# falfab/orb_slam_cuda

Measured on AMD Instinct MI355X. Metric: frames/s ORB extract+match, 1241×376 mono nFeatures=2000; achieved HBM GB/s, higher is better.
Workload: dtype u8

## Files before the change

### orb_slam_cuda_amd/csrc/orbx_blur.hip

```cpp
#include "orbx_device.cuh"

namespace orbx {

#ifndef ORBX_BLUR_TH
#define ORBX_BLUR_TH 48
#endif
#ifndef ORBX_BLUR_TW
#define ORBX_BLUR_TW 128
#endif
constexpr int kBlurTWs = 64, kBlurTHs = 32;

typedef unsigned short us2_t __attribute__((ext_vector_type(2)));
__device__ __forceinline__ uint32_t dot4(uint32_t px, uint32_t taps, uint32_t acc) {
  return __builtin_amdgcn_udot4(px, taps, acc, false);
}
__device__ __forceinline__ uint32_t dot2(uint32_t pair, uint32_t taps, uint32_t acc) {
  return __builtin_amdgcn_udot2(__builtin_bit_cast(us2_t, pair), __builtin_bit_cast(us2_t, taps), acc, false);
}

template <int kBlurTW, int kBlurTH>
__global__ __launch_bounds__(256) void blur_kernel(ExtractParams P, LevelPtrs lp, const int2* __restrict__ rtab,
                                                   int tiles, int ntiles, unsigned magic, uint8_t* __restrict__ blur) {
  constexpr int kBlurInW = kBlurTW + 32;
  constexpr int kBlurPairs = (kBlurTH + 6 + 1) / 2;
  __shared__ __attribute__((aligned(16))) uint8_t in[kBlurPairs * 2][kBlurInW];
  __shared__ __attribute__((aligned(16))) uint32_t tmp[kBlurPairs][kBlurTW];
  const int wg = xcd_remap(blockIdx.x + blockIdx.y * gridDim.x, gridDim.x * gridDim.y);
  const int f = magic ? (int)__umulhi((unsigned)wg, magic) : wg / ntiles, tid = threadIdx.x;
  const int e = rtab[tiles + wg - f * ntiles].x;
  const int l = e & 15, x0 = (e >> 4) & 0xFFF, y0 = e >> 16;
  const LevelGeom& g = P.lv[l];
  const int W = g.w, H = g.h;
  const uint8_t* S = lp.base[l] + f * lp.fstride[l];
  const int pitch = lp.pitch[l];
  typedef unsigned int u32x4 __attribute__((ext_vector_type(4)));
  constexpr int kChunks = kBlurInW / 16, kItems = (kBlurTH + 6) * kChunks, kPer = (kItems + 255) / 256;
  if (lp.aligned16[l]) {
    const int xmax = min(pitch, (W + 15) & ~15) - 16;
    u32x4 v[kPer];
#pragma unroll
    for (int q = 0; q < kPer; ++q) {
      const int i = min(tid + 256 * q, kItems - 1);
      const int r = i / kChunks, ch = i - r * kChunks;
      const int gy = reflect101(min(max(y0 + r - 3, -(H - 1)), 2 * H - 2), H);
      const int gx = min(max(x0 - 16 + ch * 16, 0), xmax);
      v[q] = *(const u32x4*)(S + (long long)gy * pitch + gx);
    }
#pragma unroll
    for (int q = 0; q < kPer; ++q) {
      const int i = min(tid + 256 * q, kItems - 1);
      const int r = i / kChunks, ch = i - r * kChunks;
      *(u32x4*)&in[r][ch * 16] = v[q];
    }
    const bool left = x0 == 0, right = x0 + kBlurTW + 3 > W;
    if (left || right) {
      __syncthreads();
      for (int i = tid; i < (kBlurTH + 6) * 6; i += 256) {
        const int r = i / 6, kk = i - r * 6;
        int x = kk < 3 ? -1 - kk : W + kk - 3;
        if ((kk < 3 && !left) || (kk >= 3 && !right) || x - x0 + 16 >= kBlurInW) continue;
        in[r][x - x0 + 16] = in[r][reflect101(x, W) - x0 + 16];
      }
    }
  } else {
    u32x4 v[kPer];
    bool direct[kPer];
    int gys[kPer];
#pragma unroll
    for (int q = 0; q < kPer; ++q) {
      const int i = min(tid + 256 * q, kItems - 1);
      const int r = i / kChunks, ch = i - r * kChunks;
      gys[q] = reflect101(min(max(y0 + r - 3, -(H - 1)), 2 * H - 2), H);
      const int gx = x0 - 16 + ch * 16;
      const uint8_t* src = S + (long long)gys[q] * pitch + gx;
      direct[q] = gx >= 0 && gx + 16 <= W && (((uintptr_t)src) & 15) == 0;
      v[q] = *(const u32x4*)(direct[q] ? src : S);
    }
#pragma unroll
    for (int q = 0; q < kPer; ++q) {
      const int i = min(tid + 256 * q, kItems - 1);
      const int r = i / kChunks, ch = i - r * kChunks;
      *(u32x4*)&in[r][ch * 16] = v[q];
    }
#pragma unroll
    for (int q = 0; q < kPer; ++q) {
      if (direct[q]) continue;
      const int i = min(tid + 256 * q, kItems - 1);
      const int r = i / kChunks, ch = i - r * kChunks;
      const int gx = x0 - 16 + ch * 16;
      const uint8_t* src = S + (long long)gys[q] * pitch;
#pragma unroll
      for (int k = 0; k < 16; ++k) {
        const int xx = min(max(gx + k, -(W - 1)), 2 * W - 2);
        in[r][ch * 16 + k] = src[reflect101(xx, W)];
      }
    }
  }
  __syncthreads();
  const int* k = P.gauss;
  const uint32_t kA0 = (k[0] << 8) | (k[1] << 16) | (k[2] << 24), kB0 = k[3] | (k[4] << 8) | (k[5] << 16) | (k[6] << 24);
  const uint32_t kA1 = (k[0] << 16) | (k[1] << 24), kB1 = k[2] | (k[3] << 8) | (k[4] << 16) | (k[5] << 24), kC1 = k[6];
  const uint32_t kA2 = k[0] << 24, kB2 = k[1] | (k[2] << 8) | (k[3] << 16) | (k[4] << 24), kC2 = k[5] | (k[6] << 8);
  const uint32_t kB3 = k[0] | (k[1] << 8) | (k[2] << 16) | (k[3] << 24), kC3 = k[4] | (k[5] << 8) | (k[6] << 16);
  const int opairs = (min(kBlurTH, H - y0) + 1) >> 1;
  for (int i = tid; i < min(kBlurPairs, opairs + 3) * (kBlurTW / 4); i += 256) {
    const int pr = i / (kBlurTW / 4), x = (i - pr * (kBlurTW / 4)) * 4;
    uint32_t o[2][4];
#pragma unroll
    for (int h = 0; h < 2; ++h) {
      const uint32_t* row = (const uint32_t*)in[2 * pr + h];
      const uint32_t A = row[(x + 12) >> 2], B = row[(x + 16) >> 2], C = row[(x + 20) >> 2];
      o[h][0] = dot4(B, kB0, dot4(A, kA0, 0));
      o[h][1] = dot4(C, kC1, dot4(B, kB1, dot4(A, kA1, 0)));
      o[h][2] = dot4(C, kC2, dot4(B, kB2, dot4(A, kA2, 0)));
      o[h][3] = dot4(C, kC3, dot4(B, kB3, 0));
    }
    *(uint4*)&tmp[pr][x] = make_uint4(o[0][0] | (o[1][0] << 16), o[0][1] | (o[1][1] << 16),
                                      o[0][2] | (o[1][2] << 16), o[0][3] | (o[1][3] << 16));
  }
  __syncthreads();
  const uint32_t t01 = k[0] | (k[1] << 16), t23 = k[2] | (k[3] << 16), t45 = k[4] | (k[5] << 16), t6 = k[6];
  const uint32_t u0 = k[0] << 16, u12 = k[1] | (k[2] << 16), u34 = k[3] | (k[4] << 16), u56 = k[5] | (k[6] << 16);
  uint8_t* D = blur + g.off + f * g.plane;
  for (int i = tid; i < opairs * (kBlurTW / 4); i += 256) {
    const int rp = i / (kBlurTW / 4), cx = (i - rp * (kBlurTW / 4)) * 4;
    const uint4 q0 = *(const uint4*)&tmp[rp][cx], q1 = *(const uint4*)&tmp[rp + 1][cx];
    const uint4 q2 = *(const uint4*)&tmp[rp + 2][cx], q3 = *(const uint4*)&tmp[rp + 3][cx];
    const uint32_t P0[4] = {q0.x, q0.y, q0.z, q0.w}, P1[4] = {q1.x, q1.y, q1.z, q1.w};
    const uint32_t P2[4] = {q2.x, q2.y, q2.z, q2.w}, P3[4] = {q3.x, q3.y, q3.z, q3.w};
    int va[4], vb[4];
#pragma unroll
    for (int q = 0; q < 4; ++q) {
      const uint32_t a = dot2(P3[q], t6, dot2(P2[q], t45, dot2(P1[q], t23, dot2(P0[q], t01, 1u << 15))));
      const uint32_t b = dot2(P3[q], u56, dot2(P2[q], u34, dot2(P1[q], u12, dot2(P0[q], u0, 1u << 15))));
      va[q] = min((int)(a >> 16), 255);
      vb[q] = min((int)(b >> 16), 255);
    }
    const uint32_t pa = pack4_u8(va[0], va[1], va[2], va[3]), pb = pack4_u8(vb[0], vb[1], vb[2], vb[3]);
    const int x = x0 + cx;
#pragma unroll
    for (int h = 0; h < 2; ++h) {
      const int y = y0 + 2 * rp + h;
      if (y >= H) break;
      const uint32_t packed = h ? pb : pa;
      uint8_t* dst = D + (long long)y * g.pitch + x;
      if (x + 4 <= W) {
        *(uint32_t*)dst = packed;
      } else {
        for (int q = 0; q < 4 && x + q < W; ++q) dst[q] = (uint8_t)(packed >> (8 * q));
      }
    }
  }
}

void blur_tile_dims(int small, int* tw, int* th) {
  *tw = small ? kBlurTWs : ORBX_BLUR_TW;
  *th = small ? kBlurTHs : ORBX_BLUR_TH;
}

int launch_blur(const ExtractParams& P, const LevelPtrs& lp, const int2* rtab, uint8_t* blur, int batch,
                hipStream_t s) {
  static const int cus = [] {
    int dev = 0, n = 256;
    (void)hipGetDevice(&dev);
    (void)hipDeviceGetAttribute(&n, hipDeviceAttributeMultiprocessorCount, dev);
    return n;
  }();
  if ((long long)P.blur_ntiles[0] * batch >= 2ll * cus)
    hipLaunchKernelGGL((blur_kernel<ORBX_BLUR_TW, ORBX_BLUR_TH>), dim3(P.blur_ntiles[0], batch), dim3(256), 0, s, P,
                       lp, rtab, P.blur_tiles[0], P.blur_ntiles[0], P.blur_magic[0], blur);
  else
    hipLaunchKernelGGL((blur_kernel<kBlurTWs, kBlurTHs>), dim3(P.blur_ntiles[1], batch), dim3(256), 0, s, P, lp,
                       rtab, P.blur_tiles[1], P.blur_ntiles[1], P.blur_magic[1], blur);
  return hipGetLastError() == hipSuccess ? ORBX_OK : ORBX_EDEVICE;
}

}
```

### orb_slam_cuda_amd/csrc/orbx_host.hip

```cpp
#include <hip/hip_runtime.h>

#include <algorithm>
#include <atomic>
#include <chrono>
#include <condition_variable>
#include <cfloat>
#include <cstdarg>
#include <climits>
#include <cmath>
#include <cstdio>
#include <cstdlib>
#include <cstring>
#include <mutex>
#include <string>
#include <thread>
#include <vector>

#include "orbx_internal.h"
#include "orbx_sincosf.h"

namespace orbx {

__global__ __launch_bounds__(256) void copy2d_kernel(uint8_t* __restrict__ d, size_t dp, const uint8_t* __restrict__ s,
                                                     size_t sp, size_t w, size_t rows) {
  const size_t cpr = (w + 15) / 16, total = cpr * rows;
  for (size_t i = blockIdx.x * 256ull + threadIdx.x; i < total; i += (size_t)gridDim.x * 256) {
    const size_t r = i / cpr, c = (i - r * cpr) * 16;
    const uint8_t* src = s + r * sp + c;
    uint8_t* dst = d + r * dp + c;
    if (c + 16 <= w) {
      *(uint4*)dst = *(const uint4*)src;
    } else {
      for (size_t k = 0; k < 16 && c + k < w; ++k) dst[k] = src[k];
    }
  }
}
size_t quadtree_lds_bytes(const ExtractParams& P);
size_t quadtree_legacy_lds_bytes(const ExtractParams& P);
size_t quadtree_sorted_lds_bytes(const ExtractParams& P, int big);
int quadtree_sorted_ownmax(const ExtractParams& P, int big, size_t budget);
extern const void* quadtree_kernel_ptr(const ExtractParams& P);
size_t pyr_band_lds_bytes(const ExtractParams& P);
void blur_tile_dims(int small, int* tw, int* th);
extern const void* pyr_band_kernel_ptr();
extern int pyr_band_occupancy(size_t lds);
}

using namespace orbx;

static size_t out_desc_off(int cap_frame) { return (16 + (size_t)cap_frame * sizeof(orbx_kp) + 15) & ~(size_t)15; }

static thread_local std::string g_err;
static int fail(int code, const char* fmt, ...) {
  char buf[512];
  va_list ap;
  va_start(ap, fmt);
  vsnprintf(buf, sizeof buf, fmt, ap);
  va_end(ap);
  g_err = buf;
  return code;
}
#define HIP_OK(expr)                                                                        \
  do {                                                                                      \
    hipError_t e_ = (expr);                                                                 \
    if (e_ != hipSuccess) return fail(ORBX_EDEVICE, "%s: %s", #expr, hipGetErrorString(e_)); \
  } while (0)

namespace {

inline int cv_round(float v) { return (int)lrintf(v); }
inline int cv_floor(float v) { int i = (int)v; return i - (i > v); }
inline short sat_short(int v) { return (short)std::min(std::max(v, (int)SHRT_MIN), (int)SHRT_MAX); }

struct DeviceBuf {
  void* p = nullptr;
  size_t n = 0;
  ~DeviceBuf() { if (p) (void)hipFree(p); }
  int alloc(size_t bytes) {
    if (p) { (void)hipFree(p); p = nullptr; }
    n = bytes;
    if (!bytes) return ORBX_OK;
    if (hipMalloc(&p, bytes) != hipSuccess) return fail(ORBX_ENOMEM, "hipMalloc(%zu) failed", bytes);
    return ORBX_OK;
  }
  template <class T> T* as() const { return (T*)p; }
};

struct Plan {
  int W = 0, H = 0, B = 0;
  ExtractParams P{};
  std::vector<CellGeom> cells;
  std::vector<int2> rtab;
  DeviceBuf pyr, blur, rtab_d, cells_d, umax_d, slots, cell_counts, qkeys, qcounts, qties, qscratch, qnscratch,
      err;
};

}

struct orbx_extractor {
  orbx_config cfg{};
  std::vector<float> scale, inv_scale, sigma2, inv_sigma2;
  std::vector<int> nfeat;
  int umax[16];
  Plan plan;
  hipStream_t stream = nullptr;
  DeviceBuf d_in, d_out;
  void* h_in = nullptr;
  void* h_out = nullptr;
  size_t h_in_bytes = 0, h_out_bytes = 0;
  hipGraphExec_t graph = nullptr;
  int graph_w = 0, graph_h = 0;
  bool graph_hp = false;
  bool last_single = false;
  bool last_empty = false;
  int warm_w = 0, warm_h = 0;
  int last_batch = 0;
  const uint8_t* last_frames = nullptr;
  size_t last_fpitch = 0, last_rstride = 0;
  bool timing = false;
  hipEvent_t ev[6] = {};
  void* user_ev[ORBX_STAGE_EVENTS] = {};
  bool has_user_ev = false;
  WsOrder ws;
  bool host_pyr = false;
  bool host_pyr_valid = false;
  void* h_pyr = nullptr;
  size_t h_pyr_bytes = 0;
  long long h_pyr_off[kMaxLevels] = {};
  hipStream_t pstream = nullptr;
  hipEvent_t pev[2] = {};
  std::vector<float> prof_t[4];
  char order[6] = {};
  std::mutex mu;
};

WsOrder* orbx::extractor_ws(orbx_handle h) { return h ? &h->ws : nullptr; }

static void compute_scales(orbx_extractor* h) {
  const orbx_config& c = h->cfg;
  const int L = c.nlevels;
  h->scale.assign(L, 1.f);
  h->sigma2.assign(L, 1.f);
  for (int i = 1; i < L; i++) {
    h->scale[i] = h->scale[i - 1] * c.scale_factor;
    h->sigma2[i] = h->scale[i] * h->scale[i];
  }
  h->inv_scale.resize(L);
  h->inv_sigma2.resize(L);
  for (int i = 0; i < L; i++) {
    h->inv_scale[i] = 1.0f / h->scale[i];
    h->inv_sigma2[i] = 1.0f / h->sigma2[i];
  }
  h->nfeat.assign(L, 0);
  const float factor = 1.0f / c.scale_factor;
  float nDesired = c.nfeatures * (1 - factor) / (1 - (float)pow((double)factor, (double)L));
  int sum = 0;
  for (int l = 0; l < L - 1; l++) {
    h->nfeat[l] = cv_round(nDesired);
    sum += h->nfeat[l];
    nDesired *= factor;
  }
  h->nfeat[L - 1] = std::max(c.nfeatures - sum, 0);
  const int HP = kHalfPatch;
  int v, v0;
  const int vmax = cv_floor(HP * sqrtf(2.f) / 2 + 1);
  const int vmin = (int)std::ceil(HP * sqrtf(2.f) / 2);
  const double hp2 = HP * HP;
  for (v = 0; v <= vmax; ++v) h->umax[v] = (int)lrint(sqrt(hp2 - v * v));
  for (v = HP, v0 = 0; v >= vmin; --v) {
    while (h->umax[v0] == h->umax[v0 + 1]) ++v0;
    h->umax[v] = v0;
    ++v0;
  }
  if (c.scale_mode == ORBX_SCALE_F) {
    for (int l = 0; l < L; ++l) {
      const unsigned vw = (unsigned)std::ceil(c.width * std::pow(0.8408964, l));
      h->scale[l] = ((float)c.width) / vw;
      h->inv_scale[l] = ((float)vw) / c.width;
    }
  }
}

static void gaussian7(int k[7]) {
  float cf[7];
  double sum = 0;
  for (int i = 0; i < 7; ++i) {
    const double x = i - 3.0;
    cf[i] = (float)std::exp(-0.5 / (2.0 * 2.0) * x * x);
    sum += cf[i];
  }
  sum = 1. / sum;
  for (int i = 0; i < 7; ++i) cf[i] = (float)(cf[i] * sum);
  for (int i = 0; i < 7; ++i) k[i] = cv_round(cf[i] * 256.f);
}

static void resize_tables(int sw, int sh, int dw, int dh, std::vector<int2>& xt, std::vector<int2>& yt,
// ... 241 lines not shown
      code |= (uint32_t)bit << (2 * (Dh - 1 - j) + 1);
    }
    t[(size_t)g.boxW + y] = code;
  }
  *bits = (Dh << 8) | ((R + 2 * Dh) << 16);
  return true;
}

static int build_plan(orbx_extractor* h, int W, int Hh, int B) {
  Plan& pl = h->plan;
  const orbx_config& c = h->cfg;
  const int L = c.nlevels;
  ExtractParams P{};
  P.L = L;
  P.B = B;
  const int ini = std::min(std::max(c.ini_th_fast, 0), 255), mn = std::min(std::max(c.min_th_fast, 0), 255);
  P.t_ini = ini;
  P.t_min = mn;
  P.t_low = std::min(ini, mn);
  P.pattern_upstream = c.pattern_mode == ORBX_PATTERN_UPSTREAM;
  gaussian7(P.gauss);
  pl.cells.clear();
  pl.rtab.clear();
  long long lvl_off = 0;
  int slot = 0, kbase = 0, maxnodes = 0, maxcells = 0;
  for (int l = 0; l < L; ++l) {
    LevelGeom& g = P.lv[l];
    const float inv = h->inv_scale[l];
    g.w = cv_round((float)W * inv);
    g.h = cv_round((float)Hh * inv);
    if (g.w > kMaxLevelDim || g.h > kMaxLevelDim)
      return fail(ORBX_EINVAL, "level %d is %dx%d; at most %d px per side", l, g.w, g.h, kMaxLevelDim);
    g.pitch = (g.w + 63) & ~63;
    g.plane = (long long)g.h * g.pitch;
    g.minBX = kEdgeThreshold - 3;
    g.minBY = g.minBX;
    g.maxBX = g.w - kEdgeThreshold + 3;
    g.maxBY = g.h - kEdgeThreshold + 3;
    const float width = (float)(g.maxBX - g.minBX), height = (float)(g.maxBY - g.minBY);
    g.nCols = (int)(width / kGridW);
    g.nRows = (int)(height / kGridW);
    if (g.nCols < 1 || g.nRows < 1)
      return fail(ORBX_EINVAL,
                  "level %d (%dx%d) is smaller than one %d-px FAST cell inside the %d-px border; "
                  "the reference divides by zero here (src/ORBextractor.cc:1144-1147)",
                  l, g.w, g.h, kGridW, kEdgeThreshold);
    g.wCell = (int)std::ceil(width / g.nCols);
    g.hCell = (int)std::ceil(height / g.nRows);
    if (g.wCell + 6 > kMaxRoi - 1 || g.hCell + 6 > kMaxRoi - 1)
      return fail(ORBX_EINVAL, "level %d cell %dx%d exceeds the ROI tile", l, g.wCell, g.hCell);
    g.cell0 = (int)pl.cells.size();
    g.slot0 = slot;
    for (int i = 0; i < g.nRows; i++) {
      const float iniY = g.minBY + i * g.hCell;
      float maxY = iniY + g.hCell + 6;
      const bool skipRow = iniY >= g.maxBY - 3;
      if (maxY > g.maxBY) maxY = g.maxBY;
      for (int j = 0; j < g.nCols; j++) {
        const float iniX = g.minBX + j * g.wCell;
        float maxX = iniX + g.wCell + 6;
        const bool skip = skipRow || iniX >= g.maxBX - 6;
        if (maxX > g.maxBX) maxX = g.maxBX;
        CellGeom cg{};
        cg.level = (int16_t)l;
        cg.c0 = (int16_t)(int)iniX;
        cg.r0 = (int16_t)(int)iniY;
        cg.c1 = (int16_t)(int)maxX;
        cg.r1 = (int16_t)(int)maxY;
        const int bw = cg.c1 - cg.c0 - 6, bh = cg.r1 - cg.r0 - 6;
        cg.cap = (skip || bw <= 0 || bh <= 0) ? 0 : (int16_t)(((bw + 1) / 2) * ((bh + 1) / 2));
        if (cg.cap) {
          P.fast_rh_max = std::max(P.fast_rh_max, cg.r1 - cg.r0);
          P.fast_bw_max = std::max(P.fast_bw_max, bw);
          P.fast_bh_max = std::max(P.fast_bh_max, bh);
        }
        cg.pitch = l == 0 ? 0 : g.pitch;
        cg.row_off = l == 0 ? cg.r0 : (int)(lvl_off + (long long)cg.r0 * g.pitch);
        cg.fstride = l == 0 ? 0 : (int)g.plane;
        cg.geo = (g.h - 1 - cg.r0) | (((g.w + 15) & ~15) << 16);
        pl.cells.push_back(cg);
      }
    }
    g.ncells = (int)pl.cells.size() - g.cell0;
    int stride = 1;
    for (int c = g.cell0; c < (int)pl.cells.size(); ++c) stride = std::max(stride, (int)pl.cells[c].cap);
    for (int c = g.cell0; c < (int)pl.cells.size(); ++c) pl.cells[c].slot_off = slot + (c - g.cell0) * stride;
    g.slot_stride = stride;
    slot += g.ncells * stride;
    g.nslots = slot - g.slot0;
    maxcells = std::max(maxcells, g.ncells);
    g.N = h->nfeat[l];
    g.boxW = g.maxBX - g.minBX;
    g.boxH = g.maxBY - g.minBY;
    g.nIni = (int)roundf(static_cast<float>(g.boxW) / g.boxH);
    if (g.nIni < 1) return fail(ORBX_EINVAL, "level %d: nIni = 0 (image taller than 1.5x its width)", l);
    g.hX = static_cast<float>(g.boxW) / g.nIni;
    g.kcap = std::max(g.N + 3, g.nIni);
    g.kbase = kbase;
    kbase += (g.kcap + kKpGroup - 1) / kKpGroup * kKpGroup;
    maxnodes = std::max(maxnodes, g.kcap + 4);
    g.scale = h->scale[l];
    g.size = (float)(int)(kPatchSize * h->scale[l]);
    g.off = lvl_off;
    lvl_off += (long long)B * g.plane;
    if (l >= 1) {
      std::vector<int2> xt, yt;
      resize_tables(P.lv[l - 1].w, P.lv[l - 1].h, g.w, g.h, xt, yt, &g.xmax, &g.area2x);
      for (int x0 = 0; x0 < g.w; x0 += 256) {
        const int xe = std::min(x0 + 255, g.w - 1);
        const int lo = g.area2x ? 2 * x0 : xt[x0].x, hi = g.area2x ? 2 * xe + 1 : xt[xe].x + 1;
        if (hi - (lo & ~15) + 16 > 576)
          return fail(ORBX_EINVAL, "scaleFactor %g too large for the pyramid tile (max 2.0)", c.scale_factor);
      }
      for (int y0 = 0; y0 < g.h; y0 += 16) {
        const int ye = std::min(y0 + 15, g.h - 1);
        const int lo = g.area2x ? 2 * y0 : (yt[y0].x & 0xFFFF), hi = g.area2x ? 2 * ye + 1 : (yt[ye].x >> 16);
        if (hi - lo + 1 > 36)
          return fail(ORBX_EINVAL, "scaleFactor %g too large for the pyramid tile (max 2.0)", c.scale_factor);
      }
      g.xtab = (int)pl.rtab.size();
      pl.rtab.insert(pl.rtab.end(), xt.begin(), xt.end());
      g.ytab = (int)pl.rtab.size();
      pl.rtab.insert(pl.rtab.end(), yt.begin(), yt.end());
      g.xtab2 = (int)pl.rtab.size();
      for (int dx = 0; dx < g.w; ++dx) {
        int2 e = xt[dx];
        if (g.area2x) e = make_int2(2 * dx, 0);
        else if (dx >= g.xmax) e.y = 2048;
        pl.rtab.push_back(e);
      }
    }
  }
  P.qt_tabmax = 0;
  P.qt_nbmax = 0;
  for (int l = 0; l < L; ++l) {
    LevelGeom& g = P.lv[l];
    std::vector<uint32_t> t;
    int bits = 0;
    g.qt_tab = -1;
    if (qt_code_tables(g, t, &bits)) {
      g.qt_tab = (int)pl.rtab.size() * 2;
      g.qt_dims = g.boxW | (g.boxH << 16);
      g.qt_bits = bits;
      if (t.size() & 1) t.push_back(0u);
      for (size_t i = 0; i < t.size(); i += 2) pl.rtab.push_back(make_int2((int)t[i], (int)t[i + 1]));
      P.qt_tabmax = std::max(P.qt_tabmax, g.boxW + g.boxH);
      P.qt_nbmax = std::max(P.qt_nbmax, 1 << ((bits >> 16) & 0xFF));
    }
  }
  if (lvl_off > INT_MAX)
    return fail(ORBX_EINVAL, "max_batch %d: the pyramid planes take %lld bytes, over 2 GiB", B, lvl_off);
  plan_band_pyramid(P, pl.rtab);
  for (int v = 0; v < 2; ++v) {
    int tw = 0, th = 0;
    blur_tile_dims(v, &tw, &th);
    P.blur_tiles[v] = (int)pl.rtab.size();
    for (int l = 0; l < L; ++l)
      for (int y0 = 0; y0 < P.lv[l].h; y0 += th)
        for (int x0 = 0; x0 < P.lv[l].w; x0 += tw) pl.rtab.push_back(make_int2(l | (x0 << 4) | (y0 << 16), 0));
    P.blur_ntiles[v] = (int)pl.rtab.size() - P.blur_tiles[v];
    const unsigned long long d = (unsigned long long)P.blur_ntiles[v];
    P.blur_magic[v] = 0u;
    if (d > 1) {
      const unsigned long long m = ((1ull << 32) + d - 1) / d, e = m * d - (1ull << 32);
      if (d * (unsigned long long)B * e < (1ull << 32)) P.blur_magic[v] = (unsigned)m;
    }
  }
  if (maxnodes > 65000) return fail(ORBX_EINVAL, "nfeatures too large for the quadtree node table");
  P.slots_per_frame = slot;
  P.ncells_total = (int)pl.cells.size();
  {
    const unsigned long long d = (unsigned long long)P.ncells_total;
    P.ncells_magic = 0u;
    if (d > 1) {
      const unsigned long long m = ((1ull << 32) + d - 1) / d, e = m * d - (1ull << 32);
      if (d * (unsigned long long)B * e < (1ull << 32)) P.ncells_magic = (unsigned)m;
    }
  }
  P.kp_per_frame = kbase;
  P.maxnodes = maxnodes;
  int sn = 1;
  while (sn < maxnodes) sn <<= 1;
  P.sortn = sn;
  P.max_cells_level = maxcells;
  P.kcap_lds = 0;
  {
    const char* e = getenv("ORBX_QT_GENERIC");
    P.qt_lean = maxnodes < 16384 && !(e && e[0] == '1');
    const char* so = getenv("ORBX_QT_SORTED");
    P.qt_sorted = P.qt_lean && P.qt_nbmax > 0 && !(so && so[0] == '0');
  }
  {
#ifndef ORBX_QT_LDS_KB
#define ORBX_QT_LDS_KB 80
#endif
    const size_t base = quadtree_legacy_lds_bytes(P);
    size_t small = ORBX_QT_LDS_KB * 1024, big = 160 * 1024 - 512;
    if (const char* e = getenv("ORBX_QT_LDS_KB")) small = (size_t)std::max(32, atoi(e)) * 1024;
    P.qt_big = base + 16 * 1024 > small ? 1 : 0;
    const size_t budget = P.qt_big ? big : small;
    P.kcap_lds = base < budget ? (int)((budget - base) / 6) & ~15 : 0;
    if (P.qt_sorted) {
      P.qt_ownmax = quadtree_sorted_ownmax(P, P.qt_big, budget);
      if (!P.qt_ownmax || quadtree_sorted_lds_bytes(P, P.qt_big) > budget) P.qt_sorted = 0;
    }
    if (maxnodes > 2 * (P.qt_big ? 1024 : kQtThreads)) P.qt_sorted = 0;
    if (getenv("ORBX_PLAN_INFO"))
      fprintf(stderr,
              "plan %dx%d B %d: quadtree LDS legacy %zu sorted %zu (budget %zu) sorted %d big %d maxnodes %d "
              "nbmax %d tabmax %d ownmax %d\n",
              W, Hh, B, base, P.qt_nbmax ? quadtree_sorted_lds_bytes(P, P.qt_big) : (size_t)0, budget, P.qt_sorted,
              P.qt_big, maxnodes, P.qt_nbmax, P.qt_tabmax, P.qt_ownmax);
  }
  pl.P = P;
  pl.W = W;
  pl.H = Hh;
  pl.B = B;
  int rc;
  if ((rc = pl.pyr.alloc((size_t)lvl_off))) return rc;
  if ((rc = pl.blur.alloc((size_t)lvl_off))) return rc;
  if ((rc = pl.rtab_d.alloc(std::max<size_t>(pl.rtab.size(), 1) * sizeof(int2)))) return rc;
  if ((rc = pl.cells_d.alloc(pl.cells.size() * sizeof(CellGeom)))) return rc;
  if ((rc = pl.umax_d.alloc(16 * sizeof(int)))) return rc;
  if ((rc = pl.slots.alloc((size_t)B * slot * 4 + 4 + 4 * 96))) return rc;
  if ((rc = pl.cell_counts.alloc((size_t)B * P.ncells_total * 4))) return rc;
  if ((rc = pl.qkeys.alloc((size_t)B * P.kp_per_frame * 4))) return rc;
  if ((rc = pl.qcounts.alloc((size_t)B * L * 4 + 4 * kMaxLevels))) return rc;
  if ((rc = pl.qties.alloc((size_t)B * L * 16))) return rc;
  if ((rc = pl.qscratch.alloc((size_t)B * slot * 4 + 4))) return rc;
  if ((rc = pl.qnscratch.alloc((size_t)B * slot * 2 + 4))) return rc;
  if ((rc = pl.err.alloc(16))) return rc;
  HIP_OK(hipMemcpy(pl.rtab_d.p, pl.rtab.data(), pl.rtab.size() * sizeof(int2), hipMemcpyHostToDevice));
  HIP_OK(hipMemcpy(pl.cells_d.p, pl.cells.data(), pl.cells.size() * sizeof(CellGeom), hipMemcpyHostToDevice));
  HIP_OK(hipMemcpy(pl.umax_d.p, h->umax, 16 * sizeof(int), hipMemcpyHostToDevice));
  HIP_OK(hipMemset(pl.err.p, 0, 16));
  if (P.pyr_fused && getenv("ORBX_PYR_PROF") && getenv("ORBX_PYR_PROF")[0] == '1')
    for (int i = 0; i < P.pyr_nplans; ++i)
      fprintf(stderr, "pyr plan %d: %d bands x %d column tiles, lds %d + %d + %d, cost %d\n", i,
              P.pyr_plan[i].nbands, P.pyr_plan[i].nct, P.pyr_plan[i].lds_a, P.pyr_plan[i].lds_b, P.pyr_plan[i].lds_y,
              P.pyr_plan[i].cost);
  if (P.pyr_fused) {
    size_t mx = 0;
    for (int i = 0; i < P.pyr_nplans; ++i) {
      ExtractParams Q = P;
      select_pyr_plan(Q, i);
      mx = std::max(mx, pyr_band_lds_bytes(Q));
    }
    if (raise_lds_limit(pyr_band_kernel_ptr(), mx))
      return fail(ORBX_EDEVICE, "LDS limit of pyr_band_kernel: %s", hipGetErrorString(hipGetLastError()));
    for (int i = 0; i < P.pyr_nplans; ++i) {
      ExtractParams Q = P;
      select_pyr_plan(Q, i);
      pl.P.pyr_plan[i].occ = pyr_band_occupancy(pyr_band_lds_bytes(Q));
      if (getenv("ORBX_PYR_PROF") && getenv("ORBX_PYR_PROF")[0] == '1')
        fprintf(stderr, "pyr plan %d: %d workgroups per CU\n", i, pl.P.pyr_plan[i].occ);
    }
  }
  if (raise_lds_limit(quadtree_kernel_ptr(P), quadtree_lds_bytes(P)))
    return fail(ORBX_EDEVICE, "LDS limit of quadtree_kernel: %s", hipGetErrorString(hipGetLastError()));
  return ORBX_OK;
}

static ExtractBuffers buffers_of(const Plan& pl) {
  ExtractBuffers X;
  X.pyr = pl.pyr.as<uint8_t>();
  X.blur = pl.blur.as<uint8_t>();
  X.rtab = pl.rtab_d.as<int2>();
  X.cells = pl.cells_d.as<CellGeom>();
  X.umax = pl.umax_d.as<int>();
  X.slots = pl.slots.as<uint32_t>();
  X.cell_counts = pl.cell_counts.as<int>();
  X.qkeys = pl.qkeys.as<uint32_t>();
  X.qcounts = pl.qcounts.as<int>();
  X.qties = pl.qties.as<int>();
  X.qscratch = pl.qscratch.as<uint32_t>();
  X.qnode_scratch = pl.qnscratch.as<uint16_t>();
  X.qscratch_per_fl = 0;
  X.err = pl.err.as<int>();
  return X;
}

int orbx::extractor_pyramid(orbx_handle h, int frame0, int n, LevelPtrs* lp, int* w, int* hgt, float* scale,
                            float* inv_scale, int* L) {
  if (!h) return fail(ORBX_EINVAL, "null extractor handle");
  if (frame0 < 0 || n < 1 || frame0 + n > h->last_batch || !h->last_frames)
    return fail(ORBX_EINVAL, "frames [%d, %d) not in the extractor's last extraction (%d frames)", frame0,
                frame0 + n, h->last_batch);
  const ExtractParams& P = h->plan.P;
  const ExtractBuffers X = buffers_of(h->plan);
  *L = P.L;
  for (int l = 0; l < P.L; ++l) {
    const LevelGeom& g = P.lv[l];
    if (l == 0) {
      lp->base[0] = h->last_frames + (long long)frame0 * h->last_fpitch;
      lp->fstride[0] = (long long)h->last_fpitch;
      lp->pitch[0] = (int)h->last_rstride;
    } else {
      lp->base[l] = X.pyr + g.off + (long long)frame0 * g.plane;
      lp->fstride[l] = g.plane;
      lp->pitch[l] = g.pitch;
    }
    lp->aligned16[l] = 0;
    w[l] = g.w;
    hgt[l] = g.h;
    scale[l] = h->scale[l];
    inv_scale[l] = h->inv_scale[l];
  }
  return ORBX_OK;
}

int orbx::extractor_last_output(orbx_handle h, const int** d_count, const orbx_kp** d_kps, const uint8_t** d_desc,
                                int* cap) {
  if (!h) return fail(ORBX_EINVAL, "null extractor handle");
  if (h->last_empty) {
// ... 765 lines not shown
```

Baseline: 183,900.

## Replace LDS-tiled Gaussian blur with per-wave register strips using DPP shifts

Rewrites the separable 7-tap blur so each wavefront processes a 248-pixel-wide vertical strip. Rows are streamed through a rotating register window of buffer loads, the vertical pass uses packed 16-bit adds and multiplies, and the horizontal pass pulls neighbour columns with DPP lane shifts instead of staging through LDS. Border reflection is handled by per-lane offsets and masked buffer stores, and the host table now lists column strips with row counts, packed four per workgroup. This removes LDS traffic and barriers, at the cost of overlapping halo lanes, more per-lane loads and a different occupancy and work-split profile.

```diff
diff --git a/orb_slam_cuda_amd/csrc/orbx_blur.hip b/orb_slam_cuda_amd/csrc/orbx_blur.hip
--- a/orb_slam_cuda_amd/csrc/orbx_blur.hip
+++ b/orb_slam_cuda_amd/csrc/orbx_blur.hip
@@ -2,160 +2,161 @@
 
 namespace orbx {
 
-#ifndef ORBX_BLUR_TH
-#define ORBX_BLUR_TH 48
+constexpr int kBlurStrip = 4 * 62;
+#ifndef ORBX_BLUR_R
+#define ORBX_BLUR_R 32
 #endif
-#ifndef ORBX_BLUR_TW
-#define ORBX_BLUR_TW 128
+#ifndef ORBX_BLUR_RS
+#define ORBX_BLUR_RS 4
 #endif
-constexpr int kBlurTWs = 64, kBlurTHs = 32;
+constexpr int kBlurR = ORBX_BLUR_R, kBlurRs = ORBX_BLUR_RS;
 
 typedef unsigned short us2_t __attribute__((ext_vector_type(2)));
-__device__ __forceinline__ uint32_t dot4(uint32_t px, uint32_t taps, uint32_t acc) {
-  return __builtin_amdgcn_udot4(px, taps, acc, false);
+__device__ __forceinline__ uint32_t dot2(us2_t pair, uint32_t taps, uint32_t acc) {
+  return __builtin_amdgcn_udot2(pair, __builtin_bit_cast(us2_t, taps), acc, false);
 }
-__device__ __forceinline__ uint32_t dot2(uint32_t pair, uint32_t taps, uint32_t acc) {
-  return __builtin_amdgcn_udot2(__builtin_bit_cast(us2_t, pair), __builtin_bit_cast(us2_t, taps), acc, false);
+__device__ __forceinline__ us2_t from_lane_below(us2_t v) {
+  return __builtin_bit_cast(us2_t, __builtin_amdgcn_mov_dpp(__builtin_bit_cast(int, v), 0x138, 0xf, 0xf, false));
+}
+__device__ __forceinline__ us2_t from_lane_above(us2_t v) {
+  return __builtin_bit_cast(us2_t, __builtin_amdgcn_mov_dpp(__builtin_bit_cast(int, v), 0x130, 0xf, 0xf, false));
 }
 
-template <int kBlurTW, int kBlurTH>
-__global__ __launch_bounds__(256) void blur_kernel(ExtractParams P, LevelPtrs lp, const int2* __restrict__ rtab,
-                                                   int tiles, int ntiles, unsigned magic, uint8_t* __restrict__ blur) {
-  constexpr int kBlurInW = kBlurTW + 32;
-  constexpr int kBlurPairs = (kBlurTH + 6 + 1) / 2;
-  __shared__ __attribute__((aligned(16))) uint8_t in[kBlurPairs * 2][kBlurInW];
-  __shared__ __attribute__((aligned(16))) uint32_t tmp[kBlurPairs][kBlurTW];
-  const int wg = xcd_remap(blockIdx.x + blockIdx.y * gridDim.x, gridDim.x * gridDim.y);
-  const int f = magic ? (int)__umulhi((unsigned)wg, magic) : wg / ntiles, tid = threadIdx.x;
-  const int e = rtab[tiles + wg - f * ntiles].x;
-  const int l = e & 15, x0 = (e >> 4) & 0xFFF, y0 = e >> 16;
-  const LevelGeom& g = P.lv[l];
-  const int W = g.w, H = g.h;
-  const uint8_t* S = lp.base[l] + f * lp.fstride[l];
-  const int pitch = lp.pitch[l];
-  typedef unsigned int u32x4 __attribute__((ext_vector_type(4)));
-  constexpr int kChunks = kBlurInW / 16, kItems = (kBlurTH + 6) * kChunks, kPer = (kItems + 255) / 256;
-  if (lp.aligned16[l]) {
-    const int xmax = min(pitch, (W + 15) & ~15) - 16;
-    u32x4 v[kPer];
+template <int MODE, bool TAIL>
+__device__ __forceinline__ void blur_strip(const int* __restrict__ k, int W, int H, int x0, int y0, int rows,
+                                           const uint8_t* S, int pitch, uint8_t* D, int dpitch, long long dplane) {
+  constexpr int kRaw = MODE == 0 ? 1 : MODE == 1 ? 2 : 4;
+  const int lane = threadIdx.x & 63;
+  const int c = x0 - 4 + 4 * lane;
+  const int srange = (H - 1) * pitch + min(pitch, (W + 15) & ~15);
+  const __amdgpu_buffer_rsrc_t srs = __builtin_amdgcn_make_buffer_rsrc((void*)S, (short)0, srange, 0x00020000);
+  int voff[kRaw];
+  uint32_t sel = 0;
+  if constexpr (MODE == 0) {
+    voff[0] = c;
+  } else {
+    int sx[4], lo = W;
 #pragma unroll
-    for (int q = 0; q < kPer; ++q) {
-      const int i = min(tid + 256 * q, kItems - 1);
-      const int r = i / kChunks, ch = i - r * kChunks;
-      const int gy = reflect101(min(max(y0 + r - 3, -(H - 1)), 2 * H - 2), H);
-      const int gx = min(max(x0 - 16 + ch * 16, 0), xmax);
-      v[q] = *(const u32x4*)(S + (long long)gy * pitch + gx);
+    for (int j = 0; j < 4; ++j) {
+      sx[j] = reflect101_clamped(c + j, W);
+      lo = min(lo, sx[j]);
     }
+    if constexpr (MODE == 1) {
+      const int a = lo & ~3;
 #pragma unroll
-    for (int q = 0; q < kPer; ++q) {
-      const int i = min(tid + 256 * q, kItems - 1);
-      const int r = i / kChunks, ch = i - r * kChunks;
-      *(u32x4*)&in[r][ch * 16] = v[q];
-    }
-    const bool left = x0 == 0, right = x0 + kBlurTW + 3 > W;
-    if (left || right) {
-      __syncthreads();
-      for (int i = tid; i < (kBlurTH + 6) * 6; i += 256) {
-        const int r = i / 6, kk = i - r * 6;
-        int x = kk < 3 ? -1 - kk : W + kk - 3;
-        if ((kk < 3 && !left) || (kk >= 3 && !right) || x - x0 + 16 >= kBlurInW) continue;
-        in[r][x - x0 + 16] = in[r][reflect101(x, W) - x0 + 16];
-      }
-    }
-  } else {
-    u32x4 v[kPer];
-    bool direct[kPer];
-    int gys[kPer];
+      for (int j = 0; j < 4; ++j) sel |= (uint32_t)min(sx[j] - a, 7) << (8 * j);
+      voff[0] = a;
+      voff[1] = min(a + 4, (W - 1) & ~3);
+    } else {
 #pragma unroll
-    for (int q = 0; q < kPer; ++q) {
-      const int i = min(tid + 256 * q, kItems - 1);
-      const int r = i / kChunks, ch = i - r * kChunks;
-      gys[q] = reflect101(min(max(y0 + r - 3, -(H - 1)), 2 * H - 2), H);
-      const int gx = x0 - 16 + ch * 16;
-      const uint8_t* src = S + (long long)gys[q] * pitch + gx;
-      direct[q] = gx >= 0 && gx + 16 <= W && (((uintptr_t)src) & 15) == 0;
-      v[q] = *(const u32x4*)(direct[q] ? src : S);
-    }
-#pragma unroll
-    for (int q = 0; q < kPer; ++q) {
-      const int i = min(tid + 256 * q, kItems - 1);
-      const int r = i / kChunks, ch = i - r * kChunks;
-      *(u32x4*)&in[r][ch * 16] = v[q];
-    }
-#pragma unroll
-    for (int q = 0; q < kPer; ++q) {
-      if (direct[q]) continue;
-      const int i = min(tid + 256 * q, kItems - 1);
-      const int r = i / kChunks, ch = i - r * kChunks;
-      const int gx = x0 - 16 + ch * 16;
-      const uint8_t* src = S + (long long)gys[q] * pitch;
-#pragma unroll
-      for (int k = 0; k < 16; ++k) {
-        const int xx = min(max(gx + k, -(W - 1)), 2 * W - 2);
-        in[r][ch * 16 + k] = src[reflect101(xx, W)];
-      }
+      for (int j = 0; j < 4; ++j) voff[j] = sx[j];
     }
   }
-  __syncthreads();
-  const int* k = P.gauss;
-  const uint32_t kA0 = (k[0] << 8) | (k[1] << 16) | (k[2] << 24), kB0 = k[3] | (k[4] << 8) | (k[5] << 16) | (k[6] << 24);
-  const uint32_t kA1 = (k[0] << 16) | (k[1] << 24), kB1 = k[2] | (k[3] << 8) | (k[4] << 16) | (k[5] << 24), kC1 = k[6];
-  const uint32_t kA2 = k[0] << 24, kB2 = k[1] | (k[2] << 8) | (k[3] << 16) | (k[4] << 24), kC2 = k[5] | (k[6] << 8);
-  const uint32_t kB3 = k[0] | (k[1] << 8) | (k[2] << 16) | (k[3] << 24), kC3 = k[4] | (k[5] << 8) | (k[6] << 16);
-  const int opairs = (min(kBlurTH, H - y0) + 1) >> 1;
-  for (int i = tid; i < min(kBlurPairs, opairs + 3) * (kBlurTW / 4); i += 256) {
-    const int pr = i / (kBlurTW / 4), x = (i - pr * (kBlurTW / 4)) * 4;
-    uint32_t o[2][4];
+  struct Raw {
+    uint32_t v[kRaw];
+  };
+  auto issue = [&](int r) {
+    const int soff = reflect101_clamped(y0 - 3 + r, H) * pitch;
+    Raw q;
 #pragma unroll
-    for (int h = 0; h < 2; ++h) {
-      const uint32_t* row = (const uint32_t*)in[2 * pr + h];
-      const uint32_t A = row[(x + 12) >> 2], B = row[(x + 16) >> 2], C = row[(x + 20) >> 2];
-      o[h][0] = dot4(B, kB0, dot4(A, kA0, 0));
-      o[h][1] = dot4(C, kC1, dot4(B, kB1, dot4(A, kA1, 0)));
-      o[h][2] = dot4(C, kC2, dot4(B, kB2, dot4(A, kA2, 0)));
-      o[h][3] = dot4(C, kC3, dot4(B, kB3, 0));
-    }
-    *(uint4*)&tmp[pr][x] = make_uint4(o[0][0] | (o[1][0] << 16), o[0][1] | (o[1][1] << 16),
-                                      o[0][2] | (o[1][2] << 16), o[0][3] | (o[1][3] << 16));
+    for (int j = 0; j < kRaw; ++j)
+      q.v[j] = MODE == 2 ? (uint32_t)__builtin_amdgcn_raw_buffer_load_b8(srs, voff[j], soff, 0)
+                         : (uint32_t)__builtin_amdgcn_raw_buffer_load_b32(srs, voff[j], soff, 0);
+    return q;
+  };
+  auto pixels = [&](const Raw& q) -> uint32_t {
+    if constexpr (MODE == 0) return q.v[0];
+    else if constexpr (MODE == 1) return __builtin_amdgcn_perm(q.v[1], q.v[0], sel);
+    else return q.v[0] | (q.v[1] << 8) | (q.v[2] << 16) | (q.v[3] << 24);
+  };
+  const us2_t k0 = {(unsigned short)k[0], (unsigned short)k[0]}, k1 = {(unsigned short)k[1], (unsigned short)k[1]};
+  const us2_t k2 = {(unsigned short)k[2], (unsigned short)k[2]}, k3 = {(unsigned short)k[3], (unsigned short)k[3]};
+  const uint32_t t_0 = k[0] << 16, t01 = k[0] | (k[1] << 16), t12 = k[1] | (k[2] << 16), t23 = k[2] | (k[3] << 16);
+  const uint32_t t34 = k[3] | (k[4] << 16), t45 = k[4] | (k[5] << 16), t56 = k[5] | (k[6] << 16), t6_ = k[6];
+  const int nsrc = rows + 6;
+  Raw q[7];
+  us2_t wl[7], wh[7];
+  auto unpack = [&](int slot) {
+    const uint32_t p = pixels(q[slot]);
+    wl[slot] = __builtin_bit_cast(us2_t, __builtin_amdgcn_perm(0u, p, 0x0c010c00u));
+    wh[slot] = __builtin_bit_cast(us2_t, __builtin_amdgcn_perm(0u, p, 0x0c030c02u));
+  };
+#pragma unroll
+  for (int r = 0; r < 7; ++r) q[r] = issue(r);
+#pragma unroll
+  for (int r = 0; r < 6; ++r) {
+    unpack(r);
+    q[r] = issue(min(r + 7, nsrc - 1));
   }
-  __syncthreads();
-  const uint32_t t01 = k[0] | (k[1] << 16), t23 = k[2] | (k[3] << 16), t45 = k[4] | (k[5] << 16), t6 = k[6];
-  const uint32_t u0 = k[0] << 16, u12 = k[1] | (k[2] << 16), u34 = k[3] | (k[4] << 16), u56 = k[5] | (k[6] << 16);
-  uint8_t* D = blur + g.off + f * g.plane;
-  for (int i = tid; i < opairs * (kBlurTW / 4); i += 256) {
-    const int rp = i / (kBlurTW / 4), cx = (i - rp * (kBlurTW / 4)) * 4;
-    const uint4 q0 = *(const uint4*)&tmp[rp][cx], q1 = *(const uint4*)&tmp[rp + 1][cx];
-    const uint4 q2 = *(const uint4*)&tmp[rp + 2][cx], q3 = *(const uint4*)&tmp[rp + 3][cx];
-    const uint32_t P0[4] = {q0.x, q0.y, q0.z, q0.w}, P1[4] = {q1.x, q1.y, q1.z, q1.w};
-    const uint32_t P2[4] = {q2.x, q2.y, q2.z, q2.w}, P3[4] = {q3.x, q3.y, q3.z, q3.w};
-    int va[4], vb[4];
+  const __amdgpu_buffer_rsrc_t drs = __builtin_amdgcn_make_buffer_rsrc((void*)D, (short)0, (int)dplane, 0x00020000);
+  const bool owner = lane >= 1 && lane <= 62 && c < W;
+  constexpr int kDrop = 0x40000000;
+  const int st4 = owner && c + 4 <= W ? c : kDrop;
+  int st1[3];
 #pragma unroll
-    for (int q = 0; q < 4; ++q) {
-      const uint32_t a = dot2(P3[q], t6, dot2(P2[q], t45, dot2(P1[q], t23, dot2(P0[q], t01, 1u << 15))));
-      const uint32_t b = dot2(P3[q], u56, dot2(P2[q], u34, dot2(P1[q], u12, dot2(P0[q], u0, 1u << 15))));
-      va[q] = min((int)(a >> 16), 255);
-      vb[q] = min((int)(b >> 16), 255);
-    }
-    const uint32_t pa = pack4_u8(va[0], va[1], va[2], va[3]), pb = pack4_u8(vb[0], vb[1], vb[2], vb[3]);
-    const int x = x0 + cx;
+  for (int b = 0; b < 3; ++b) st1[b] = owner && c + 4 > W && c + b < W ? c + b : kDrop;
+#pragma unroll 1
+  for (int i0 = 0; i0 < rows; i0 += 7) {
 #pragma unroll
-    for (int h = 0; h < 2; ++h) {
-      const int y = y0 + 2 * rp + h;
-      if (y >= H) break;
-      const uint32_t packed = h ? pb : pa;
-      uint8_t* dst = D + (long long)y * g.pitch + x;
-      if (x + 4 <= W) {
-        *(uint32_t*)dst = packed;
-      } else {
-        for (int q = 0; q < 4 && x + q < W; ++q) dst[q] = (uint8_t)(packed >> (8 * q));
+    for (int j = 0; j < 7; ++j) {
+      const int i = i0 + j;
+      if (i >= rows) break;
+      unpack((j + 6) % 7);
+      q[(j + 6) % 7] = issue(min(i + 13, nsrc - 1));
+      const us2_t al = wl[j] + wl[(j + 6) % 7], ah = wh[j] + wh[(j + 6) % 7];
+      const us2_t bl = wl[(j + 1) % 7] + wl[(j + 5) % 7], bh = wh[(j + 1) % 7] + wh[(j + 5) % 7];
+      const us2_t cl = wl[(j + 2) % 7] + wl[(j + 4) % 7], ch = wh[(j + 2) % 7] + wh[(j + 4) % 7];
+      const us2_t vl = al * k0 + bl * k1 + cl * k2 + wl[(j + 3) % 7] * k3;
+      const us2_t vh = ah * k0 + bh * k1 + ch * k2 + wh[(j + 3) % 7] * k3;
+      const us2_t ll = from_lane_below(vl), lh = from_lane_below(vh);
+      const us2_t rl = from_lane_above(vl), rh = from_lane_above(vh);
+      const uint32_t o0 = dot2(vh, t56, dot2(vl, t34, dot2(lh, t12, dot2(ll, t_0, 1u << 15))));
+      const uint32_t o1 = dot2(rl, t6_, dot2(vh, t45, dot2(vl, t23, dot2(lh, t01, 1u << 15))));
+      const uint32_t o2 = dot2(rl, t56, dot2(vh, t34, dot2(vl, t12, dot2(lh, t_0, 1u << 15))));
+      const uint32_t o3 = dot2(rh, t6_, dot2(rl, t45, dot2(vh, t23, dot2(vl, t01, 1u << 15))));
+      const us2_t hi = {255, 255};
+      const us2_t m01 = __builtin_elementwise_min(__builtin_bit_cast(us2_t, __builtin_amdgcn_perm(o1, o0, 0x07060302u)), hi);
+      const us2_t m23 = __builtin_elementwise_min(__builtin_bit_cast(us2_t, __builtin_amdgcn_perm(o3, o2, 0x07060302u)), hi);
+      const uint32_t packed =
+          __builtin_amdgcn_perm(__builtin_bit_cast(uint32_t, m23), __builtin_bit_cast(uint32_t, m01), 0x06040200u);
+      const int soff = (y0 + i) * dpitch;
+      __builtin_amdgcn_raw_buffer_store_b32(packed, drs, st4, soff, 0);
+      if constexpr (TAIL) {
+#pragma unroll
+        for (int b = 0; b < 3; ++b)
+          __builtin_amdgcn_raw_buffer_store_b8((uint8_t)(packed >> (8 * b)), drs, st1[b], soff, 0);
       }
     }
   }
 }
 
-void blur_tile_dims(int small, int* tw, int* th) {
-  *tw = small ? kBlurTWs : ORBX_BLUR_TW;
-  *th = small ? kBlurTHs : ORBX_BLUR_TH;
+template <bool BYTES0>
+__global__ __launch_bounds__(256) void blur_kernel(ExtractParams P, LevelPtrs lp, const int2* __restrict__ rtab,
+                                                   int items, int nitems, int nwg, unsigned magic,
+                                                   uint8_t* __restrict__ blur) {
+  const int wg = xcd_remap(blockIdx.x + blockIdx.y * gridDim.x, gridDim.x * gridDim.y);
+  const int f = magic ? (int)__umulhi((unsigned)wg, magic) : wg / nwg;
+  const int it = (wg - f * nwg) * 4 + __builtin_amdgcn_readfirstlane(threadIdx.x >> 6);
+  if (it >= nitems) return;
+  const int2 e = rtab[items + it];
+  const int l = e.x & 15, x0 = (e.x >> 4) & 0xFFF, y0 = e.x >> 16, rows = e.y;
+  const LevelGeom& g = P.lv[l];
+  const int W = g.w, H = g.h;
+  const uint8_t* S = lp.base[l] + f * lp.fstride[l];
+  uint8_t* D = blur + g.off + f * g.plane;
+  if (BYTES0 && l == 0)
+    blur_strip<2, true>(P.gauss, W, H, x0, y0, rows, S, lp.pitch[l], D, g.pitch, g.plane);
+  else if ((W & 3) && x0 + kBlurStrip >= W)
+    blur_strip<1, true>(P.gauss, W, H, x0, y0, rows, S, lp.pitch[l], D, g.pitch, g.plane);
+  else if (x0 == 0 || x0 + kBlurStrip + 4 > W)
+    blur_strip<1, false>(P.gauss, W, H, x0, y0, rows, S, lp.pitch[l], D, g.pitch, g.plane);
+  else
+    blur_strip<0, false>(P.gauss, W, H, x0, y0, rows, S, lp.pitch[l], D, g.pitch, g.plane);
+}
+
+void blur_strip_dims(int small, int* strip, int* rows) {
+  *strip = kBlurStrip;
+  *rows = small ? kBlurRs : kBlurR;
 }
 
 int launch_blur(const ExtractParams& P, const LevelPtrs& lp, const int2* rtab, uint8_t* blur, int batch,
@@ -166,12 +167,14 @@
     (void)hipDeviceGetAttribute(&n, hipDeviceAttributeMultiprocessorCount, dev);
     return n;
   }();
-  if ((long long)P.blur_ntiles[0] * batch >= 2ll * cus)
-    hipLaunchKernelGGL((blur_kernel<ORBX_BLUR_TW, ORBX_BLUR_TH>), dim3(P.blur_ntiles[0], batch), dim3(256), 0, s, P,
-                       lp, rtab, P.blur_tiles[0], P.blur_ntiles[0], P.blur_magic[0], blur);
+  const int v = (long long)P.blur_ntiles[0] * batch >= 8ll * cus ? 0 : 1;
+  const int nwg = (P.blur_ntiles[v] + 3) / 4;
+  if (lp.aligned16[0])
+    hipLaunchKernelGGL(blur_kernel<false>, dim3(nwg, batch), dim3(256), 0, s, P, lp, rtab, P.blur_tiles[v],
+                       P.blur_ntiles[v], nwg, P.blur_magic[v], blur);
   else
-    hipLaunchKernelGGL((blur_kernel<kBlurTWs, kBlurTHs>), dim3(P.blur_ntiles[1], batch), dim3(256), 0, s, P, lp,
-                       rtab, P.blur_tiles[1], P.blur_ntiles[1], P.blur_magic[1], blur);
+    hipLaunchKernelGGL(blur_kernel<true>, dim3(nwg, batch), dim3(256), 0, s, P, lp, rtab, P.blur_tiles[v],
+                       P.blur_ntiles[v], nwg, P.blur_magic[v], blur);
   return hipGetLastError() == hipSuccess ? ORBX_OK : ORBX_EDEVICE;
 }
 
diff --git a/orb_slam_cuda_amd/csrc/orbx_host.hip b/orb_slam_cuda_amd/csrc/orbx_host.hip
--- a/orb_slam_cuda_amd/csrc/orbx_host.hip
+++ b/orb_slam_cuda_amd/csrc/orbx_host.hip
@@ -41,7 +41,7 @@
 int quadtree_sorted_ownmax(const ExtractParams& P, int big, size_t budget);
 extern const void* quadtree_kernel_ptr(const ExtractParams& P);
 size_t pyr_band_lds_bytes(const ExtractParams& P);
-void blur_tile_dims(int small, int* tw, int* th);
+void blur_strip_dims(int small, int* strip, int* rows);
 extern const void* pyr_band_kernel_ptr();
 extern int pyr_band_occupancy(size_t lds);
 }
@@ -589,14 +589,15 @@
     return fail(ORBX_EINVAL, "max_batch %d: the pyramid planes take %lld bytes, over 2 GiB", B, lvl_off);
   plan_band_pyramid(P, pl.rtab);
   for (int v = 0; v < 2; ++v) {
-    int tw = 0, th = 0;
-    blur_tile_dims(v, &tw, &th);
+    int sw = 0, R = 0;
+    blur_strip_dims(v, &sw, &R);
     P.blur_tiles[v] = (int)pl.rtab.size();
     for (int l = 0; l < L; ++l)
-      for (int y0 = 0; y0 < P.lv[l].h; y0 += th)
-        for (int x0 = 0; x0 < P.lv[l].w; x0 += tw) pl.rtab.push_back(make_int2(l | (x0 << 4) | (y0 << 16), 0));
+      for (int x0 = 0; x0 < P.lv[l].w; x0 += sw)
+        for (int y0 = 0; y0 < P.lv[l].h; y0 += R)
+          pl.rtab.push_back(make_int2(l | (x0 << 4) | (y0 << 16), std::min(R, P.lv[l].h - y0)));
     P.blur_ntiles[v] = (int)pl.rtab.size() - P.blur_tiles[v];
-    const unsigned long long d = (unsigned long long)P.blur_ntiles[v];
+    const unsigned long long d = (unsigned long long)(P.blur_ntiles[v] + 3) / 4;
     P.blur_magic[v] = 0u;
     if (d > 1) {
       const unsigned long long m = ((1ull << 32) + d - 1) / d, e = m * d - (1ull << 32);
```

Result: faster. 189,800 (median of 6 runs) (+3.2%).
